# BioJulia/Kmers.jl

Measured on NVIDIA B200. Metric: canonical 31-mers+hash/sec, higher is better.
Workload: dtype u64

## Files before the change

### kmers.jl_b200/csrc/api.cu

```cuda
#include <algorithm>
#include <cstdio>
#include <cstring>
#include <new>
#include <vector>

#include "fourbit.h"
#include "plan.h"

namespace kmc {

int32_t fail_cuda(kmc_ctx *ctx, cudaError_t e, const char *what)
{
    if (ctx) {
        char buf[512];
        snprintf(buf, sizeof buf, "%s: %s (%s)", what, cudaGetErrorName(e), cudaGetErrorString(e));
        ctx->last_error = buf;
    }
    return -static_cast<int32_t>(e);
}

int32_t fail(kmc_ctx *ctx, int32_t code, const char *msg)
{
    if (ctx) ctx->last_error = msg;
    return code;
}

ExtractLaunchFn get_launcher(const Geometry &ge, int mode, bool hash, bool ragged)
{
    switch (ge.n_limbs) {
    case 1: return get_extract_launcher_n1(ge.nx, mode, hash, ragged);
    case 2: return get_extract_launcher_n2(ge.nx, mode, hash, ragged);
    case 3: return get_extract_launcher_n3(ge.nx, mode, hash, ragged);
    case 4: return get_extract_launcher_n4(ge.nx, mode, hash, ragged);
    }
    return nullptr;
}

ExtractLaunchFn get_digest_launcher(const Geometry &ge, int mode, bool hash, bool ragged)
{
    switch (ge.n_limbs) {
    case 1: return get_digest_launcher_n1(ge.nx, mode, hash, ragged);
    case 2: return get_digest_launcher_n2(ge.nx, mode, hash, ragged);
    }
    return nullptr;
}

namespace {

bool aligned32(const void *p) { return (reinterpret_cast<uintptr_t>(p) & 31) == 0; }

__global__ void fill_uniform_offsets_kernel(uint64_t *out, uint64_t n_plus_1, uint64_t step)
{
    uint64_t i = static_cast<uint64_t>(blockIdx.x) * blockDim.x + threadIdx.x;
    if (i < n_plus_1) out[i] = i * step;
}

}

cudaError_t fill_uniform_offsets(uint64_t *out, uint64_t n_plus_1, uint64_t step, cudaStream_t stream)
{
    fill_uniform_offsets_kernel<<<static_cast<unsigned>((n_plus_1 + 255) / 256), 256, 0, stream>>>(out, n_plus_1, step);
    return cudaGetLastError();
}

int32_t check_common(kmc_ctx *ctx, const kmc_seqs *s, int32_t k)
{
    if (!ctx) return KMC_E_BAD_ARG;
    if (!s) return fail(ctx, KMC_E_BAD_ARG, "kmc_seqs is NULL");
    if (k < 1) return fail(ctx, KMC_E_BAD_K, "K must be at least 1");
    if (k > KMC_MAX_K) return fail(ctx, KMC_E_BAD_K, "K exceeds KMC_MAX_K (128)");
    if (s->src_bits != 2 && s->src_bits != 4 && s->src_bits != 8)
        return fail(ctx, KMC_E_BAD_ARG, "src_bits must be 2, 4 (LongSequence words) or 8 (ASCII bytes)");
    if (s->n_seqs > 0 && s->words == nullptr && s->n_words > 0) return fail(ctx, KMC_E_BAD_ARG, "words is NULL");
    return KMC_OK;
}

uint64_t layout_scratch_bytes(const kmc_seqs *s)
{
    if (s->seq_len == nullptr) return 0;
    const uint64_t n = s->n_seqs;
    return 4 * round_up((n + 1) * 8, 256) + round_up(scan_tmp_elems(n) * 8, 256) +
           round_up((tiles_upper_bound(s) + 1) * 8, 256);
}

int32_t plan_layout(kmc_ctx *ctx, const kmc_seqs *s, int k, const Geometry &ge, cudaStream_t stream,
                    const KnownTotals &known, Scratch &scratch, Layout *L)
{
    L->uniform_len = (s->seq_len == nullptr);
    L->uniform_off = (s->seq_word_offset == nullptr);
    const uint64_t G = static_cast<uint64_t>(ge.g);
    if (L->uniform_len) {
        L->wpr = s->uniform_len >= static_cast<uint64_t>(k) ? s->uniform_len - k + 1 : 0;
        L->total = L->wpr * s->n_seqs;
        L->gprm = (L->wpr % G == 0) ? L->wpr / G : (L->wpr + G - 1) / G + 1;
        if (s->n_seqs == 1) L->gprm = (L->wpr + G - 1) / G;
        L->items = L->gprm * s->n_seqs;
        return KMC_OK;
    }
    const uint64_t n = s->n_seqs;
    uint64_t *cnt = static_cast<uint64_t *>(scratch.take((n + 1) * 8));
    uint64_t *win_off = static_cast<uint64_t *>(scratch.take((n + 1) * 8));
    uint64_t *slots = static_cast<uint64_t *>(scratch.take((n + 1) * 8));
    uint64_t *item_off = static_cast<uint64_t *>(scratch.take((n + 1) * 8));
    uint64_t *tmp = static_cast<uint64_t *>(scratch.take(scan_tmp_elems(n) * 8));
    if (!cnt || !win_off || !slots || !item_off || !tmp) return fail(ctx, KMC_E_BAD_ARG, "internal: scratch window too small");
    CU(window_counts(s->seq_len, n, k, cnt, stream));
    CU(inclusive_offsets_u64(cnt, win_off, n, tmp, stream));
    CU(group_slots(win_off, n, ge.g, slots, stream));
    CU(inclusive_offsets_u64(slots, item_off, n, tmp, stream));
    L->win_off = win_off;
    L->item_off = item_off;
    L->wpr = 0;
    L->gprm = 1;
    if (known.valid) {
        L->total = known.windows;
        L->items = known.items;
    } else {
        uint64_t h[2] = {0, 0};
        CU(cudaMemcpyAsync(&h[0], win_off + n, sizeof(uint64_t), cudaMemcpyDeviceToHost, stream));
        CU(cudaMemcpyAsync(&h[1], item_off + n, sizeof(uint64_t), cudaMemcpyDeviceToHost, stream));
        CU(cudaStreamSynchronize(stream));
        L->total = h[0];
        L->items = h[1];
    }
    const uint64_t tiles = (L->items + kTileItems - 1) / kTileItems;
    if (tiles) {
        uint64_t *tile_first = static_cast<uint64_t *>(scratch.take((tiles + 1) * 8));
        if (!tile_first) return fail(ctx, KMC_E_BAD_ARG, "internal: scratch window too small");
        CU(tile_first_reads(item_off, n, kTileItems, tiles, tile_first, stream));
        L->tile_first = tile_first;
    }
    return KMC_OK;
}

ExtractParams base_params(const kmc_seqs *s, int k, const Geometry &ge, const Layout &L, uint64_t unit_bias)
{
    ExtractParams p;
    memset(&p, 0, sizeof p);
    p.w32 = reinterpret_cast<const uint32_t *>(s->words);
    p.nw32 = static_cast<int64_t>(s->n_words) * 2;
    p.unit_bits = 64;
    p.unit_bias = unit_bias;
    p.first = s->first_symbol_offset;
    p.k = k;
    p.s0 = ge.s0;
    p.head_mask = ge.head_mask;
    p.n_seqs = s->n_seqs;
    p.items = L.items;
    p.stride_units = s->uniform_stride_words;
    p.wpr = L.wpr;
    p.gprm = L.gprm;
    p.seq_unit_off = s->seq_word_offset;
    p.win_off = L.win_off;
    p.item_off = L.item_off;
    p.tile_first = L.tile_first;
    return p;
}

int32_t bind_outputs(kmc_ctx *ctx, const kmc_out *out, int mode, uint32_t flags, ExtractParams *p)
{
    const bool hash = (flags & KMC_HASH_FX) != 0;
    const bool aos = (flags & KMC_AOS) != 0;
    const bool want_index = (mode == KMC_UNAMBIG);
    if (!out->a) return fail(ctx, KMC_E_BAD_ARG, "out.a is NULL");
    if (mode == KMC_FWRV && !aos && !out->b) return fail(ctx, KMC_E_BAD_ARG, "out.b is NULL (FWRV, SoA)");
    if (hash && !out->hash) return fail(ctx, KMC_E_BAD_ARG, "out.hash is NULL (KMC_HASH_FX)");
    if (want_index && !aos && !out->index) return fail(ctx, KMC_E_BAD_ARG, "out.index is NULL (UNAMBIG, SoA)");
    p->out_a = out->a;
    p->out_b = out->b;
    p->out_hash = hash ? out->hash : nullptr;
    p->out_index = want_index ? (aos ? reinterpret_cast<int64_t *>(out->a) : out->index) : nullptr;
    p->index_base = out->index_base;
    p->aos = aos ? 1u : 0u;
    p->vec_ok = aligned32(out->a) && (!p->out_b || aligned32(p->out_b)) && (!p->out_hash || aligned32(p->out_hash)) &&
                (!p->out_index || aligned32(p->out_index));
    return KMC_OK;
}

uint64_t extract_scratch_bytes(const kmc_seqs *s, int k, int mode)
{
    if (s->src_bits != 2) return fourbit_scratch_bytes(s, k, mode);
    return layout_scratch_bytes(s) + 256;
}

int32_t extract_device(kmc_ctx *ctx, const kmc_seqs *s, int32_t k, int32_t mode, uint32_t flags, const kmc_out *out,
                       kmc_result *res, cudaStream_t stream, const KnownTotals &known, uint64_t unit_bias, bool sync,
                       Scratch &scratch)
{
    const Geometry ge = geometry(k);
    const bool hash = (flags & KMC_HASH_FX) != 0;
    const int kmode = (mode == KMC_UNAMBIG) ? MODE_FW : mode;

    if (sync) CU(cudaEventRecord(ctx->ev_k0, stream));
    if ((flags & KMC_AOS) && (mode == KMC_FWRV || mode == KMC_UNAMBIG) && ge.n_limbs == 1 && !s->seq_len && !s->seq_word_offset) {
        const Geometry g2 = geometry(k, 2, kAosGroup);
        Layout L2;
        int32_t st2 = plan_layout(ctx, s, k, g2, stream, known, scratch, &L2);
        if (st2) return st2;
        AosLaunchFn afn = get_aos_launcher_n1(g2.nx, mode == KMC_FWRV, hash);
        if (afn && L2.total > 0 && L2.total <= out->capacity) {
            ExtractParams p2 = base_params(s, k, g2, L2, unit_bias);
            st2 = bind_outputs(ctx, out, mode, flags, &p2);
            if (st2) return st2;
            const cudaError_t e = afn(p2, stream);
            if (e == cudaSuccess) {
                res->n_written = L2.total;
                if (out->seq_out_offset) CU(fill_uniform_offsets(out->seq_out_offset, s->n_seqs + 1, L2.wpr, stream));
                if (sync) {
                    CU(cudaEventRecord(ctx->ev_k1, stream));
                    CU(cudaStreamSynchronize(stream));
                    CU(cudaEventElapsedTime(&res->kernel_ms, ctx->ev_k0, ctx->ev_k1));
                }
                return KMC_OK;
            }
            if (e != cudaErrorNotSupported) return fail_cuda(ctx, e, "launch_extract_aos");
            (void)cudaGetLastError();
        }
    }
    Layout L;
    int32_t st = plan_layout(ctx, s, k, ge, stream, known, scratch, &L);
    if (st) return st;
    res->n_written = L.total;
    if (out->seq_out_offset) {
        if (L.uniform_len)
            CU(fill_uniform_offsets(out->seq_out_offset, s->n_seqs + 1, L.wpr, stream));
        else
            CU(cudaMemcpyAsync(out->seq_out_offset, L.win_off, (s->n_seqs + 1) * sizeof(uint64_t), cudaMemcpyDeviceToDevice, stream));
    }
    if (L.total == 0) return KMC_OK;
    if (L.total > out->capacity) return fail(ctx, KMC_E_OUT_TOO_SMALL, "output capacity smaller than the number of k-mers");
    ExtractParams p = base_params(s, k, ge, L, unit_bias);
    st = bind_outputs(ctx, out, mode, flags, &p);
    if (st) return st;

    const bool fused_digest = known.digest && digest_fusable(s, ge.n_limbs, mode, flags);
    if (fused_digest) p.digest = known.digest;
    ExtractLaunchFn fn = fused_digest ? get_digest_launcher(ge, kmode, hash, !L.uniform_len) : get_launcher(ge, kmode, hash, !L.uniform_len);
    if (!fn) return fail(ctx, KMC_E_UNSUPPORTED, "no kernel for this K");
    CU(fn(p, ctx->sm_count, stream));
    if (sync) {
        CU(cudaEventRecord(ctx->ev_k1, stream));
        CU(cudaStreamSynchronize(stream));
        CU(cudaEventElapsedTime(&res->kernel_ms, ctx->ev_k0, ctx->ev_k1));
    }
    return KMC_OK;
}

int32_t ensure_scratch(kmc_ctx *ctx, uint64_t bytes)
{
    if (bytes <= ctx->scratch_bytes) return KMC_OK;
    if (ctx->scratch) {
        CU(cudaStreamSynchronize(ctx->stream));
        for (int i = 0; i < 3; ++i) CU(cudaStreamSynchronize(ctx->pipe_streams[i]));
        CU(cudaFree(ctx->scratch));
        ctx->scratch = nullptr;
        ctx->scratch_bytes = 0;
    }
    uint64_t want = bytes + bytes / 4 + 4096;
    CU(cudaMalloc(&ctx->scratch, want));
    ctx->scratch_bytes = want;
    return KMC_OK;
}

int32_t ensure_host_small(kmc_ctx *ctx)
{
    if (ctx->host_small) return KMC_OK;
    CU(cudaHostAlloc(reinterpret_cast<void **>(&ctx->host_small), 4096, cudaHostAllocDefault));
    memset(ctx->host_small, 0, 4096);
    CU(cudaMalloc(reinterpret_cast<void **>(&ctx->dev_small), 128));
    return KMC_OK;
}

}

using namespace kmc;

extern "C" {

int32_t kmc_version(void) { return KMC_VERSION; }

int32_t kmc_device_count(int32_t *n)
{
    if (!n) return KMC_E_BAD_ARG;
    int c = 0;
    cudaError_t e = cudaGetDeviceCount(&c);
    if (e != cudaSuccess) {
        *n = 0;
        return (e == cudaErrorNoDevice || e == cudaErrorInsufficientDriver) ? KMC_E_NO_DEVICE : -static_cast<int32_t>(e);
    }
    *n = c;
    return KMC_OK;
}

int32_t kmc_ctx_create(int32_t device, kmc_ctx **out)
{
    if (!out) return KMC_E_BAD_ARG;
    *out = nullptr;
    int32_t n = 0;
    int32_t st = kmc_device_count(&n);
    if (st) return st;
    if (n == 0 || device < 0 || device >= n) return KMC_E_NO_DEVICE;
    kmc_ctx *ctx = new (std::nothrow) kmc_ctx();
    if (!ctx) return KMC_E_BAD_ARG;
    ctx->device = device;
    cudaError_t e = cudaSetDevice(device);
    if (e == cudaSuccess) e = cudaDeviceGetAttribute(&ctx->sm_count, cudaDevAttrMultiProcessorCount, device);
    if (e == cudaSuccess) {
        cudaMemPoolProps props;
        memset(&props, 0, sizeof props);
        props.allocType = cudaMemAllocationTypePinned;
        props.handleTypes = cudaMemHandleTypeNone;
        props.location.type = cudaMemLocationTypeDevice;
        props.location.id = device;
        if (cudaMemPoolCreate(&ctx->pool, &props) == cudaSuccess) {
            uint64_t keep = ~0ull;
            cudaMemPoolSetAttribute(ctx->pool, cudaMemPoolAttrReleaseThreshold, &keep);
        } else {
            ctx->pool = nullptr;
        }
        (void)cudaGetLastError();
    }
    if (e == cudaSuccess) e = cudaStreamCreateWithFlags(&ctx->own_stream, cudaStreamNonBlocking);
    for (int i = 0; i < 3 && e == cudaSuccess; ++i) e = cudaStreamCreateWithFlags(&ctx->pipe_streams[i], cudaStreamNonBlocking);
    if (e == cudaSuccess) e = cudaEventCreate(&ctx->ev_begin);
    if (e == cudaSuccess) e = cudaEventCreate(&ctx->ev_end);
    if (e == cudaSuccess) e = cudaEventCreate(&ctx->ev_k0);
    if (e == cudaSuccess) e = cudaEventCreate(&ctx->ev_k1);
    if (e != cudaSuccess) {
        delete ctx;
        return -static_cast<int32_t>(e);
    }
    ctx->stream = ctx->own_stream;
    *out = ctx;
    return KMC_OK;
}

int32_t kmc_ctx_destroy(kmc_ctx *ctx)
{
    if (!ctx) return KMC_OK;
    cudaSetDevice(ctx->device);
    cudaStreamSynchronize(ctx->stream);
    if (ctx->scratch) cudaFree(ctx->scratch);
    if (ctx->host_small) cudaFreeHost(ctx->host_small);
    if (ctx->dev_small) cudaFree(ctx->dev_small);
    for (int i = 0; i < 3; ++i) {
        if (ctx->pipe_buf[i]) cudaFree(ctx->pipe_buf[i]);
        if (ctx->pipe_streams[i]) cudaStreamDestroy(ctx->pipe_streams[i]);
        if (ctx->pipe_events[i]) cudaEventDestroy(ctx->pipe_events[i]);
    }
    if (ctx->ev_begin) cudaEventDestroy(ctx->ev_begin);
    if (ctx->ev_end) cudaEventDestroy(ctx->ev_end);
    if (ctx->ev_k0) cudaEventDestroy(ctx->ev_k0);
    if (ctx->ev_k1) cudaEventDestroy(ctx->ev_k1);
    if (ctx->comm) comm_detach(ctx);
    if (ctx->own_stream) cudaStreamDestroy(ctx->own_stream);
    if (ctx->pool) cudaMemPoolDestroy(ctx->pool);
    delete ctx;
    return KMC_OK;
}

int32_t kmc_ctx_set_stream(kmc_ctx *ctx, void *cuda_stream)
{
    if (!ctx) return KMC_E_BAD_ARG;
    ctx->stream = cuda_stream ? static_cast<cudaStream_t>(cuda_stream) : ctx->own_stream;
    return KMC_OK;
}

int32_t kmc_sync(kmc_ctx *ctx)
{
    if (!ctx) return KMC_E_BAD_ARG;
    CU(cudaSetDevice(ctx->device));
    CU(cudaStreamSynchronize(ctx->stream));
    return KMC_OK;
}

int32_t kmc_trim(kmc_ctx *ctx)
{
    if (!ctx) return KMC_E_BAD_ARG;
    CU(cudaSetDevice(ctx->device));
    CU(cudaStreamSynchronize(ctx->stream));
    for (int i = 0; i < 3; ++i) CU(cudaStreamSynchronize(ctx->pipe_streams[i]));
    if (ctx->pool) CU(cudaMemPoolTrimTo(ctx->pool, 0));
    return KMC_OK;
}

const char *kmc_last_error(kmc_ctx *ctx) { return ctx ? ctx->last_error.c_str() : "kmc_ctx is NULL"; }

const char *kmc_status_string(int32_t status)
{
    switch (status) {
    case KMC_OK: return "ok";
    case KMC_E_BAD_K: return "K must be at least 1 (and at most KMC_MAX_K)";
    case KMC_E_BAD_ARG: return "bad argument";
    case KMC_E_AMBIGUOUS: return "cannot encode an uncertain symbol in a 2-bit alphabet";
    case KMC_E_OUT_TOO_SMALL: return "output buffer too small";
    case KMC_E_NO_DEVICE: return "no CUDA device";
    case KMC_E_UNSUPPORTED: return "unsupported configuration";
    case KMC_E_NCCL: return "NCCL error (or NCCL could not be loaded)";
    }
    if (status < 0) return cudaGetErrorString(static_cast<cudaError_t>(-status));
    return "unknown status";
}

int32_t kmc_device_info(kmc_ctx *ctx, int32_t *sm_count, uint64_t *total_mem, char *name, int32_t name_len)
{
    if (!ctx) return KMC_E_BAD_ARG;
    cudaDeviceProp prop;
    CU(cudaGetDeviceProperties(&prop, ctx->device));
    if (sm_count) *sm_count = prop.multiProcessorCount;
    if (total_mem) *total_mem = prop.totalGlobalMem;
    if (name && name_len > 0) {
        strncpy(name, prop.name, static_cast<size_t>(name_len) - 1);
        name[name_len - 1] = 0;
    }
    return KMC_OK;
}

int32_t kmc_malloc(kmc_ctx *ctx, uint64_t bytes, void **dptr)
{
    if (!ctx || !dptr) return KMC_E_BAD_ARG;
    CU(cudaSetDevice(ctx->device));
    CU(cudaMalloc(dptr, bytes ? bytes : 1));
    return KMC_OK;
}

int32_t kmc_free(kmc_ctx *ctx, void *dptr)
{
    if (!ctx) return KMC_E_BAD_ARG;
    if (!dptr) return KMC_OK;
    CU(cudaSetDevice(ctx->device));
    CU(cudaFree(dptr));
    return KMC_OK;
}

int32_t kmc_memset(kmc_ctx *ctx, void *dptr, int32_t value, uint64_t bytes)
{
    if (!ctx) return KMC_E_BAD_ARG;
    if (bytes == 0) return KMC_OK;
    CU(cudaSetDevice(ctx->device));
    CU(cudaMemsetAsync(dptr, value, bytes, ctx->stream));
    return KMC_OK;
}

int32_t kmc_upload(kmc_ctx *ctx, void *dptr, const void *host, uint64_t bytes)
{
    if (!ctx) return KMC_E_BAD_ARG;
    if (bytes == 0) return KMC_OK;
    CU(cudaSetDevice(ctx->device));
    CU(cudaMemcpyAsync(dptr, host, bytes, cudaMemcpyHostToDevice, ctx->stream));
    return KMC_OK;
}

int32_t kmc_download(kmc_ctx *ctx, void *host, const void *dptr, uint64_t bytes)
{
    if (!ctx) return KMC_E_BAD_ARG;
    CU(cudaSetDevice(ctx->device));
    if (bytes) CU(cudaMemcpyAsync(host, dptr, bytes, cudaMemcpyDeviceToHost, ctx->stream));
    CU(cudaStreamSynchronize(ctx->stream));
    return KMC_OK;
}

int32_t kmc_host_alloc(kmc_ctx *ctx, uint64_t bytes, void **hptr)
{
    if (!ctx || !hptr) return KMC_E_BAD_ARG;
    CU(cudaSetDevice(ctx->device));
    CU(cudaHostAlloc(hptr, bytes ? bytes : 1, cudaHostAllocDefault));
    return KMC_OK;
}

int32_t kmc_host_free(kmc_ctx *ctx, void *hptr)
{
    if (!ctx) return KMC_E_BAD_ARG;
    if (!hptr) return KMC_OK;
    CU(cudaFreeHost(hptr));
    return KMC_OK;
}

int32_t kmc_host_register(kmc_ctx *ctx, void *hptr, uint64_t bytes)
{
    if (!ctx || !hptr) return KMC_E_BAD_ARG;
    CU(cudaSetDevice(ctx->device));
    CU(cudaHostRegister(hptr, bytes, cudaHostRegisterDefault));
    return KMC_OK;
}

int32_t kmc_host_unregister(kmc_ctx *ctx, void *hptr)
{
    if (!ctx || !hptr) return KMC_E_BAD_ARG;
    CU(cudaHostUnregister(hptr));
    return KMC_OK;
}

int32_t kmc_count(kmc_ctx *ctx, const kmc_seqs *seqs, int32_t k, int32_t mode, uint64_t *n_out)
{
    int32_t st = check_common(ctx, seqs, k);
    if (st) return st;
    if (!n_out) return fail(ctx, KMC_E_BAD_ARG, "n_out is NULL");
    if (mode < KMC_FW || mode > KMC_UNAMBIG) return fail(ctx, KMC_E_BAD_ARG, "unknown mode");
    CU(cudaSetDevice(ctx->device));
    if (mode == KMC_UNAMBIG && seqs->src_bits != 2) return count_unambiguous_4bit(ctx, seqs, k, n_out, ctx->stream);
    const Geometry ge = geometry(k);
    st = ensure_scratch(ctx, layout_scratch_bytes(seqs) + 256);
    if (st) return st;
    Scratch scratch{static_cast<char *>(ctx->scratch), ctx->scratch_bytes, 0};
    Layout L;
    st = plan_layout(ctx, seqs, k, ge, ctx->stream, KnownTotals(), scratch, &L);
    if (st) return st;
    *n_out = L.total;
    return KMC_OK;
}

int32_t kmc_extract(kmc_ctx *ctx, const kmc_seqs *seqs, int32_t k, int32_t mode, uint32_t flags, const kmc_out *out,
                    kmc_result *result)
{
    int32_t st = check_common(ctx, seqs, k);
    if (st) return st;
    if (!out || !result) return fail(ctx, KMC_E_BAD_ARG, "kmc_out / kmc_result is NULL");
    if (mode < KMC_FW || mode > KMC_UNAMBIG) return fail(ctx, KMC_E_BAD_ARG, "unknown mode");
    CU(cudaSetDevice(ctx->device));
    result->n_written = 0;
    result->err_seq = result->err_pos = 0;
    result->err_sym = 0;
    result->kernel_ms = 0.f;
    if (flags & KMC_KMER4) {
        st = check_kmer4(ctx, seqs, k, mode);
        if (st) return st;
        st = ensure_scratch(ctx, kmer4_scratch_bytes(seqs));
        if (st) return st;
        Scratch scratch{static_cast<char *>(ctx->scratch), ctx->scratch_bytes, 0};
        return extract_device_kmer4(ctx, seqs, k, mode, flags, out, result, ctx->stream, KnownTotals(), 0,
                                    (flags & KMC_NO_SYNC) == 0, scratch);
    }
    if (seqs->src_bits != 2) return extract_device_4bit(ctx, seqs, k, mode, flags, out, result, ctx->stream);
    st = ensure_scratch(ctx, extract_scratch_bytes(seqs, k, mode));
    if (st) return st;
    Scratch scratch{static_cast<char *>(ctx->scratch), ctx->scratch_bytes, 0};
    return extract_device(ctx, seqs, k, mode, flags, out, result, ctx->stream, KnownTotals(), 0,
                          (flags & KMC_NO_SYNC) == 0, scratch);
}

int32_t kmc_fx_hash(kmc_ctx *ctx, const uint64_t *kmers, uint64_t n, int32_t n_limbs, uint64_t h0, uint64_t *out)
{
    if (!ctx) return KMC_E_BAD_ARG;
    if (n_limbs < 0 || n_limbs > 4) return fail(ctx, KMC_E_BAD_ARG, "n_limbs must be in 0..4");
    if (n && (!out || (n_limbs && !kmers))) return fail(ctx, KMC_E_BAD_ARG, "NULL buffer");
    CU(cudaSetDevice(ctx->device));
    CU(launch_fx_hash(kmers, n, n_limbs, h0, out, ctx->sm_count, ctx->stream));
    return KMC_OK;
}

int32_t kmc_base_hash(kmc_ctx *ctx, const uint64_t *kmers, uint64_t n, int32_t n_limbs, int32_t k, uint64_t h0, uint64_t *out)
{
    if (!ctx) return KMC_E_BAD_ARG;
    if (n_limbs < 0 || n_limbs > 4) return fail(ctx, KMC_E_BAD_ARG, "n_limbs must be in 0..4");
    if (k < 0) return fail(ctx, KMC_E_BAD_K, "K must not be negative");
    if (n && (!out || (n_limbs && !kmers))) return fail(ctx, KMC_E_BAD_ARG, "NULL buffer");
    CU(cudaSetDevice(ctx->device));
    CU(launch_base_hash(kmers, n, n_limbs, h0 ^ static_cast<uint64_t>(k), out, ctx->sm_count, ctx->stream));
    return KMC_OK;
}

namespace {
int32_t bucket_count_impl(kmc_ctx *ctx, const kmc_seqs *seqs, int32_t k, int32_t bucket_bits, uint32_t *table, uint32_t n_parts,
                          void *const *events, kmc_result *result);
}

int32_t kmc_bucket_count(kmc_ctx *ctx, const kmc_seqs *seqs, int32_t k, int32_t bucket_bits, uint32_t *table,
                         kmc_result *result)
{
    return bucket_count_impl(ctx, seqs, k, bucket_bits, table, 0, nullptr, result);
}

int32_t kmc_bucket_count_async(kmc_ctx *ctx, const kmc_seqs *seqs, int32_t k, int32_t bucket_bits, uint32_t *table,
                               uint32_t n_parts, void *const *events, kmc_result *result)
{
    if (!ctx) return KMC_E_BAD_ARG;
    if (!events || n_parts < 1 || n_parts > 32 || (n_parts & (n_parts - 1)))
        return fail(ctx, KMC_E_BAD_ARG, "n_parts must be a power of two <= 32 and events non-NULL");
    for (uint32_t i = 0; i < n_parts; ++i)
        if (!events[i]) return fail(ctx, KMC_E_BAD_ARG, "NULL event");
    return bucket_count_impl(ctx, seqs, k, bucket_bits, table, n_parts, events, result);
}

namespace {
int32_t bucket_count_impl(kmc_ctx *ctx, const kmc_seqs *seqs, int32_t k, int32_t bucket_bits, uint32_t *table, uint32_t n_parts,
                          void *const *events, kmc_result *result)
{
    int32_t st = check_common(ctx, seqs, k);
    if (st) return st;
    if (!table || !result) return fail(ctx, KMC_E_BAD_ARG, "table / result is NULL");
    if (bucket_bits < 1 || bucket_bits > 32) return fail(ctx, KMC_E_BAD_ARG, "bucket_bits must be in 1..32");
    if (seqs->src_bits != 2) return fail(ctx, KMC_E_UNSUPPORTED, "bucket count needs a 2-bit source");
    CU(cudaSetDevice(ctx->device));
    result->n_written = 0;
    result->err_seq = result->err_pos = 0;
    result->err_sym = 0;
    result->kernel_ms = 0.f;
    const Geometry ge = geometry(k);
    cudaStream_t stream = ctx->stream;
    CU(cudaEventRecord(ctx->ev_k0, stream));
    st = ensure_scratch(ctx, layout_scratch_bytes(seqs) + 256);
    if (st) return st;
    Scratch scratch{static_cast<char *>(ctx->scratch), ctx->scratch_bytes, 0};
    Layout L;
    st = plan_layout(ctx, seqs, k, ge, stream, KnownTotals(), scratch, &L);
    if (st) return st;
    result->n_written = L.total;
    auto record_all = [&]() -> int32_t {
        for (uint32_t i = 0; i < n_parts; ++i) CU(cudaEventRecord(static_cast<cudaEvent_t>(events[i]), stream));
        return KMC_OK;
    };
    if (L.total == 0) return record_all();
    ExtractParams p = base_params(seqs, k, ge, L, 0);
    p.bucket_shift = static_cast<uint32_t>(64 - bucket_bits);
    const uint64_t table_bytes = 4ull << bucket_bits;
    const bool want_binned = table_bytes > (96ull << 20) && bucket_bits <= 32;

    auto count_direct = [&](ExtractParams q, cudaStream_t s) -> int32_t {
        int32_t rc = ensure_host_small(ctx);
        if (rc) return rc;
        if (table_bytes <= (96ull << 20)) CU(warm_table(table, 1ull << bucket_bits, ctx->sm_count, warm_sink(ctx), s));
        q.bucket_table = table;
        ExtractLaunchFn fn = get_launcher(ge, MODE_BUCKETS, true, !L.uniform_len);
        if (!fn) return fail(ctx, KMC_E_UNSUPPORTED, "no kernel for this K");
        CU(fn(q, ctx->sm_count, s));
        return KMC_OK;
    };
    auto count_exact = [&](ExtractParams q, uint64_t windows, cudaStream_t s, uint32_t np, void *const *ev) -> int32_t {
        AsyncBuf ids_buf, tmp_buf, matrix_buf, offs_buf, scan_buf;
        const uint64_t n_ids = (q.items + 1) * static_cast<uint64_t>(ge.g);
        const uint64_t cells = (static_cast<uint64_t>(1) << binned_count_bin_bits(bucket_bits)) * binned_count_blocks(n_ids);
        cudaError_t e = ids_buf.alloc(ctx, round_up(n_ids * 4, 256), s);
        if (e == cudaSuccess) e = tmp_buf.alloc(ctx, round_up(n_ids * 4, 256), s);
        if (e == cudaSuccess) e = matrix_buf.alloc(ctx, (cells + 1) * 8, s);
        if (e == cudaSuccess) e = offs_buf.alloc(ctx, (cells + 2) * 8, s);
        if (e == cudaSuccess) e = scan_buf.alloc(ctx, (scan_tmp_elems(cells) + 1) * 8, s);
        if (e != cudaSuccess) {
            (void)cudaGetLastError();
            int32_t rc = count_direct(q, s);
            if (rc) return rc;
            for (uint32_t i = 0; i < np; ++i) CU(cudaEventRecord(static_cast<cudaEvent_t>(ev[i]), s));
            return KMC_OK;
        }
        q.out_a = ids_buf.as<uint64_t>();
        q.vec_ok = 1;
        ExtractLaunchFn fn = get_launcher(ge, MODE_BUCKET_IDS, true, !L.uniform_len);
        if (!fn) return fail(ctx, KMC_E_UNSUPPORTED, "no kernel for this K");
        CU(fn(q, ctx->sm_count, s));
        CU(binned_count(ids_buf.as<uint32_t>(), windows, bucket_bits, table, tmp_buf.as<uint32_t>(), matrix_buf.as<uint64_t>(),
                        offs_buf.as<uint64_t>(), scan_buf.as<uint64_t>(), ctx->sm_count, s, np, ev));
        return KMC_OK;
    };

    bool done = false;
    ExtractParams pa = p;
    if (want_binned) set_iteration_strides(pa, ge.g);
    if (want_binned && ge.n_limbs == 1 && L.uniform_len && binned_count_bin_bits(bucket_bits) == 6 && fused_bin_enabled() && pa.aligned &&
        pa.al_tail == 0 && pa.items < 0xffffffffull - kTileItems) {
        AsyncBuf bins_buf, state_buf;
        const uint64_t cap = fused_bin_capacity(L.total);
        cudaError_t e = bins_buf.alloc(ctx, fused_bin_buffer_ids(L.total) * 4, stream);
        if (e == cudaSuccess) e = state_buf.alloc(ctx, fused_bin_state_bytes(), stream);
        if (e != cudaSuccess) {
            (void)cudaGetLastError();
        } else {
            st = ensure_host_small(ctx);
            if (st) return st;
            CU(fused_bin_ids(pa, ge.nx, bucket_bits, bins_buf.as<uint32_t>(), cap, state_buf.as<unsigned long long>(), stream));
            CU(fused_bin_apply(bins_buf.as<uint32_t>(), cap, state_buf.as<unsigned long long>(), bucket_bits, table, warm_sink(ctx),
                               ctx->sm_count, stream, n_parts, events));
            done = true;
        }
    }
    if (!done && want_binned) {
        st = count_exact(p, L.total, stream, n_parts, events);
        if (st) return st;
        done = true;
    }
    if (!done) {
        st = count_direct(p, stream);
        if (st) return st;
        st = record_all();
        if (st) return st;
    }
    if (n_parts) return KMC_OK;
    CU(cudaEventRecord(ctx->ev_k1, stream));
    CU(cudaStreamSynchronize(stream));
    CU(cudaEventElapsedTime(&result->kernel_ms, ctx->ev_k0, ctx->ev_k1));
    return KMC_OK;
}
}

int32_t kmc_digest(kmc_ctx *ctx, const uint64_t *dptr, uint64_t n, uint64_t *out)
{
    if (!ctx) return KMC_E_BAD_ARG;
    if (!out || (n && !dptr)) return fail(ctx, KMC_E_BAD_ARG, "NULL buffer");
    CU(cudaSetDevice(ctx->device));
    int32_t st = ensure_scratch(ctx, 256);
    if (st) return st;
    uint64_t *acc = static_cast<uint64_t *>(ctx->scratch);
    CU(launch_digest(dptr, n, acc, ctx->sm_count, ctx->stream));
    CU(cudaMemcpyAsync(out, acc, 16, cudaMemcpyDeviceToHost, ctx->stream));
    CU(cudaStreamSynchronize(ctx->stream));
    return KMC_OK;
}

int32_t kmc_timer_begin(kmc_ctx *ctx)
{
    if (!ctx) return KMC_E_BAD_ARG;
    CU(cudaSetDevice(ctx->device));
    CU(cudaEventRecord(ctx->ev_begin, ctx->stream));
    return KMC_OK;
}

int32_t kmc_timer_end(kmc_ctx *ctx, float *ms)
{
    if (!ctx || !ms) return KMC_E_BAD_ARG;
    CU(cudaSetDevice(ctx->device));
    CU(cudaEventRecord(ctx->ev_end, ctx->stream));
    CU(cudaEventSynchronize(ctx->ev_end));
    CU(cudaEventElapsedTime(ms, ctx->ev_begin, ctx->ev_end));
    return KMC_OK;
}

int32_t kmc_store_probe(kmc_ctx *ctx, void *dptr, uint64_t bytes)
{
    if (!ctx || !dptr) return KMC_E_BAD_ARG;
    CU(cudaSetDevice(ctx->device));
    CU(launch_store_probe(dptr, bytes, ctx->sm_count, ctx->stream));
    return KMC_OK;
}

}
```

### kmers.jl_b200/csrc/buckets.cu

```cuda
#include <cstdlib>
#include <type_traits>

#include "binning.cuh"
#include "plan.h"

namespace kmc {

namespace {

__global__ void __launch_bounds__(256) warm_slice_kernel(const uint32_t *__restrict__ slice, uint64_t n_counters,
                                                         uint32_t *__restrict__ sink)
{
    const uint4 *p = reinterpret_cast<const uint4 *>(slice);
    const uint64_t n4 = n_counters / 4;
    uint32_t acc = 0;
    for (uint64_t i = static_cast<uint64_t>(blockIdx.x) * blockDim.x + threadIdx.x; i < n4;
         i += static_cast<uint64_t>(gridDim.x) * blockDim.x) {
        uint4 v;
        asm volatile("ld.global.L1::no_allocate.L2::cache_hint.v4.u32 {%0,%1,%2,%3}, [%4], %5;"
                     : "=r"(v.x), "=r"(v.y), "=r"(v.z), "=r"(v.w)
                     : "l"(p + i), "l"(0x14F0000000000000ull));
        acc |= v.x & v.y & v.z & v.w;
    }
    if (acc == 0xffffffffu) *sink = acc;
}

__global__ void __launch_bounds__(256) bin_apply_kernel(const uint32_t *__restrict__ binned, const uint64_t *__restrict__ offs,
                                                        uint64_t n_blocks, int bin, int bin_end, uint32_t *__restrict__ table)
{
    const uint64_t begin = __ldg(offs + static_cast<uint64_t>(bin) * n_blocks);
    const uint64_t end = __ldg(offs + static_cast<uint64_t>(bin_end) * n_blocks);
    const uint64_t a4 = (begin + 3) & ~3ull;
    const uint64_t tid = static_cast<uint64_t>(blockIdx.x) * blockDim.x + threadIdx.x;
    const uint64_t threads = static_cast<uint64_t>(gridDim.x) * blockDim.x;
    if (tid < a4 - begin && begin + tid < end) atomicAdd(table + binned[begin + tid], 1u);
    for (uint64_t i = a4 + tid * 4; i < end; i += threads * 4) {
        if (i + 4 <= end) {
            const uint4 v = __ldg(reinterpret_cast<const uint4 *>(binned + i));
            atomicAdd(table + v.x, 1u);
            atomicAdd(table + v.y, 1u);
            atomicAdd(table + v.z, 1u);
            atomicAdd(table + v.w, 1u);
        } else {
            for (uint64_t j = i; j < end; ++j) atomicAdd(table + binned[j], 1u);
        }
    }
}


constexpr int kStateBinEnd = binning::kTpBins;
constexpr int kStateSpill = 2 * binning::kTpBins;
constexpr int kStateWords = 2 * binning::kTpBins + 2;

struct FusedBins {
    uint32_t *binned;
    uint64_t cap;
    unsigned long long *state;
    int bin_shift;
};

template <int NX>
__global__ void __launch_bounds__(binning::kBlock, 3) bucket_bin_kernel(const ExtractParams p, const FusedBins f)
{
    using S = binning::Shape<uint32_t>;
    constexpr int G = 8, PT = S::kPerThread;
    static_assert(PT == 2 * G && S::kChunk == kTileItems * G, "a thread bins the ids of two work items per iteration");
    extern __shared__ __align__(16) unsigned char smem_raw[];
    binning::Scatter64Smem<uint32_t> &sm = *reinterpret_cast<binning::Scatter64Smem<uint32_t> *>(smem_raw);
    const uint32_t n_items = static_cast<uint32_t>(p.items);
    const uint32_t tile_base = blockIdx.x * static_cast<uint32_t>(kTileItems);
    if (p.pf_tiles) burst_prefetch<false, G, 2>(p, n_items);
    const AlignedItems<G, 2> items(p);
    const uint32_t tile_end = n_items - tile_base > static_cast<uint32_t>(kTileItems) ? tile_base + kTileItems : n_items;
    const bool inside = items.template loads_inside<NX>(p, tile_end - 1u);
    const binning::IdBin bin_of{f.bin_shift};
    constexpr int kItemsPerIter = 2 * binning::kBlock;
    auto reserve = [&](int b, uint32_t count) -> uint64_t {
        if (count == 0) return 0;
        const uint64_t at = atomicAdd(f.state + b, static_cast<unsigned long long>(count));
        if (at + count > f.cap) {
            atomicMin(f.state + kStateBinEnd + b, static_cast<unsigned long long>(at));
            return binning::kTpBins * f.cap + atomicAdd(f.state + kStateSpill, static_cast<unsigned long long>(count));
        }
        return static_cast<uint64_t>(b) * f.cap + at;
    };
    auto ids_of = [&](uint32_t item, uint32_t *key) {
        uint32_t x[NX];
        load_block_at<NX>(p, items.bit_of(item), inside, x);
        uint64_t fw[G][1], rv[G][1];
        block_kmers<1, NX, G, true, true, 2>(x, p.s0, p.head_mask, fw, rv);
#pragma unroll
        for (int j = 0; j < G; ++j) {
            const uint64_t c[1] = {fw[j][0] < rv[j][0] ? fw[j][0] : rv[j][0]};
            key[j] = static_cast<uint32_t>(fx_hash<1>(c, 0) >> p.bucket_shift);
        }
    };
#pragma unroll 1
    for (uint32_t it_base = tile_base; it_base < tile_end; it_base += kItemsPerIter) {
        uint32_t key[PT];
        if (tile_end - it_base >= static_cast<uint32_t>(kItemsPerIter)) {
            ids_of(it_base + threadIdx.x, key);
            ids_of(it_base + binning::kBlock + threadIdx.x, key + G);
            binning::scatter64_iter<uint32_t, true>(sm, key, 0xffffu, bin_of, reserve, f.binned);
        } else {
            uint32_t ok_mask = 0;
#pragma unroll
            for (int j = 0; j < PT; ++j) key[j] = 0;
            if (it_base + threadIdx.x < tile_end) {
                ids_of(it_base + threadIdx.x, key);
                ok_mask = 0xffu;
            }
            if (it_base + binning::kBlock + threadIdx.x < tile_end) {
                ids_of(it_base + binning::kBlock + threadIdx.x, key + G);
                ok_mask |= 0xff00u;
            }
            binning::scatter64_iter<uint32_t, false>(sm, key, ok_mask, bin_of, reserve, f.binned);
        }
    }
}

__device__ __forceinline__ uint4 ld_ids(const uint32_t *p)
{
    uint4 v;
    asm volatile("ld.global.nc.L1::no_allocate.L2::cache_hint.v4.u32 {%0,%1,%2,%3}, [%4], %5;"
                 : "=r"(v.x), "=r"(v.y), "=r"(v.z), "=r"(v.w)
                 : "l"(p), "l"(0x12F0000000000000ull));
    return v;
}
__device__ __forceinline__ void inc_counter(uint32_t *p)
{
    asm volatile("red.global.add.L2::cache_hint.u32 [%0], 1, %1;" ::"l"(p), "l"(0x14F0000000000000ull) : "memory");
}

__global__ void __launch_bounds__(256) bin_apply_fused_kernel(const uint32_t *__restrict__ binned, uint64_t cap,
                                                              const unsigned long long *__restrict__ state, int bin, int bin_end,
                                                              uint32_t *__restrict__ table)
{
    const uint64_t tid = static_cast<uint64_t>(blockIdx.x) * blockDim.x + threadIdx.x;
    const uint64_t step = static_cast<uint64_t>(gridDim.x) * blockDim.x * 4;
    for (int b = bin; b < bin_end; ++b) {
        const uint32_t *ids = binned + static_cast<uint64_t>(b) * cap;
        const uint64_t reserved = state[b], full_at = state[kStateBinEnd + b];
        const uint64_t n = reserved < full_at ? reserved : full_at, n4 = n & ~3ull;
        uint64_t i = tid * 4;
        uint4 v = make_uint4(0, 0, 0, 0);
        if (i < n4) v = ld_ids(ids + i);
        while (i < n4) {
            const uint64_t nxt = i + step;
            uint4 w = make_uint4(0, 0, 0, 0);
            if (nxt < n4) w = ld_ids(ids + nxt);
            inc_counter(table + v.x);
            inc_counter(table + v.y);
            inc_counter(table + v.z);
            inc_counter(table + v.w);
            v = w;
            i = nxt;
        }
        if (tid < n - n4) inc_counter(table + ids[n4 + tid]);
    }
}

__global__ void __launch_bounds__(256) spill_apply_kernel(const uint32_t *__restrict__ spill, const unsigned long long *__restrict__ state,
                                                          uint32_t *__restrict__ table)
{
    const uint64_t n = state[kStateSpill];
    for (uint64_t i = static_cast<uint64_t>(blockIdx.x) * blockDim.x + threadIdx.x; i < n; i += static_cast<uint64_t>(gridDim.x) * blockDim.x)
        atomicAdd(table + spill[i], 1u);
}

}

cudaError_t binned_count(const uint32_t *ids, uint64_t n, int bucket_bits, uint32_t *table, uint32_t *binned, uint64_t *matrix,
                         uint64_t *offs, uint64_t *scan_tmp, int sm_count, cudaStream_t stream, uint32_t n_parts, void *const *events)
{
    if (!events) n_parts = 0;
    if (n == 0) {
        for (uint32_t i = 0; i < n_parts; ++i) {
            cudaError_t e = cudaEventRecord(static_cast<cudaEvent_t>(events[i]), stream);
            if (e != cudaSuccess) return e;
        }
        return cudaSuccess;
    }
    const int p = binned_count_bin_bits(bucket_bits);
    if (bucket_bits < p) return cudaErrorInvalidValue;
    const int n_bins = 1 << p, shift = bucket_bits - p;
    const uint64_t n_blocks = binned_count_blocks(n);
    cudaError_t e = binning::partition<uint32_t>(ids, n, p, binning::IdBin{shift}, binned, matrix, offs, scan_tmp, stream);
    if (e != cudaSuccess) return e;
    const uint64_t slice = 1ull << shift;
    const int group = apply_group(2);
    uint32_t parts_done = 0;
    for (int b = 0; b < n_bins; b += group) {
        const int b_end = b + group < n_bins ? b + group : n_bins;
        warm_slice_kernel<<<static_cast<unsigned>(sm_count * 8), 256, 0, stream>>>(table + static_cast<uint64_t>(b) * slice,
                                                                                  slice * (b_end - b), reinterpret_cast<uint32_t *>(scan_tmp));
        bin_apply_kernel<<<static_cast<unsigned>(sm_count * 16), 256, 0, stream>>>(binned, offs, n_blocks, b, b_end, table);
        while (parts_done < n_parts && static_cast<uint64_t>(parts_done + 1) * n_bins <= static_cast<uint64_t>(b_end) * n_parts) {
            e = cudaEventRecord(static_cast<cudaEvent_t>(events[parts_done++]), stream);
            if (e != cudaSuccess) return e;
        }
    }
    return cudaGetLastError();
}

uint64_t fused_bin_capacity(uint64_t n_ids)
{
    const uint64_t cap = n_ids / binning::kTpBins + n_ids / (8 * binning::kTpBins) + 8192;
    return (cap + 3) & ~3ull;
}
uint64_t fused_bin_buffer_ids(uint64_t n_ids) { return binning::kTpBins * fused_bin_capacity(n_ids) + n_ids + 4096; }
uint64_t fused_bin_state_bytes() { return kStateWords * sizeof(unsigned long long); }

cudaError_t fused_bin_ids(ExtractParams p, int nx, int bucket_bits, uint32_t *binned, uint64_t cap, unsigned long long *state,
                          cudaStream_t stream)
{
    const int pbits = binned_count_bin_bits(bucket_bits);
    if (pbits != 6 || bucket_bits < pbits) return cudaErrorInvalidValue;
    const uint64_t tiles = (p.items + kTileItems - 1) / kTileItems;
    if (tiles == 0 || tiles > 0x7fffffffull || p.items >= 0xffffffffull - kTileItems) return cudaErrorInvalidConfiguration;
    set_iteration_strides(p, 8);
    if (!p.aligned || p.al_tail) return cudaErrorInvalidValue;
    p.al_magic = aligned_magic(p.gprm);
    p.pf_tiles = 0;
    if (prefetch_enabled()) {
        const uint64_t per_tile = static_cast<uint64_t>(p.nw32) * 4 / tiles + 1, t = kPfChunkBytes / per_tile;
        p.pf_tiles = static_cast<uint32_t>(t < 2 * kPfLead ? 2 * kPfLead : (t > (1u << 20) ? (1u << 20) : t));
    }
    cudaError_t e = cudaMemsetAsync(state, 0, kStateWords * sizeof(unsigned long long), stream);
    if (e == cudaSuccess) e = cudaMemsetAsync(state + kStateBinEnd, 0xff, binning::kTpBins * sizeof(unsigned long long), stream);
    if (e != cudaSuccess) return e;
    const FusedBins f{binned, cap, state, bucket_bits - pbits};
    constexpr int smem = static_cast<int>(sizeof(binning::Scatter64Smem<uint32_t>));
    auto launch = [&](auto tag) -> cudaError_t {
        constexpr int NX = decltype(tag)::value;
        cudaError_t e2 = cudaFuncSetAttribute(bucket_bin_kernel<NX>, cudaFuncAttributeMaxDynamicSharedMemorySize, smem);
        if (e2 != cudaSuccess) return e2;
        bucket_bin_kernel<NX><<<static_cast<unsigned>(tiles), binning::kBlock, smem, stream>>>(p, f);
        return cudaGetLastError();
    };
    switch (nx) {
    case 1: return launch(std::integral_constant<int, 1>());
    case 2: return launch(std::integral_constant<int, 2>());
    case 3: return launch(std::integral_constant<int, 3>());
    }
    return cudaErrorInvalidValue;
}

cudaError_t fused_bin_apply(const uint32_t *binned, uint64_t cap, const unsigned long long *state, int bucket_bits, uint32_t *table,
                            uint32_t *sink, int sm_count, cudaStream_t stream, uint32_t n_parts, void *const *events)
{
    if (!events) n_parts = 0;
    const int pbits = binned_count_bin_bits(bucket_bits);
    const int n_bins = 1 << pbits, shift = bucket_bits - pbits;
    const uint64_t slice = 1ull << shift;
    const int group = apply_group(2);
    spill_apply_kernel<<<static_cast<unsigned>(sm_count * 8), 256, 0, stream>>>(binned + static_cast<uint64_t>(n_bins) * cap, state, table);
    uint32_t parts_done = 0;
    for (int b = 0; b < n_bins; b += group) {
        const int b_end = b + group < n_bins ? b + group : n_bins;
        warm_slice_kernel<<<static_cast<unsigned>(sm_count * 8), 256, 0, stream>>>(table + static_cast<uint64_t>(b) * slice,
                                                                                  slice * (b_end - b), sink);
        bin_apply_fused_kernel<<<static_cast<unsigned>(sm_count * 16), 256, 0, stream>>>(binned, cap, state, b, b_end, table);
        while (parts_done < n_parts && static_cast<uint64_t>(parts_done + 1) * n_bins <= static_cast<uint64_t>(b_end) * n_parts) {
            cudaError_t e = cudaEventRecord(static_cast<cudaEvent_t>(events[parts_done++]), stream);
            if (e != cudaSuccess) return e;
        }
    }
    return cudaGetLastError();
}

bool fused_bin_enabled()
{
    static const bool on = [] {
        const char *e = getenv("KMC_FUSED_BIN");
        return !(e && e[0] == '0');
    }();
    return on;
}

int apply_group(int dflt)
{
    static const int env = [] {
        const char *e = getenv("KMC_APPLY_GROUP");
        const int v = e ? atoi(e) : 0;
        return v < 0 ? 0 : (v > 64 ? 64 : v);
    }();
    return env ? env : dflt;
}

cudaError_t warm_table(const uint32_t *table, uint64_t n_counters, int sm_count, uint32_t *sink, cudaStream_t stream)
{
    warm_slice_kernel<<<static_cast<unsigned>(sm_count * 8), 256, 0, stream>>>(table, n_counters, sink);
    return cudaGetLastError();
}

int binned_count_bin_bits(int bucket_bits)
{
    int p = bucket_bits - 22;
    if (p < binning::kMinBits) p = binning::kMinBits;
    if (p > binning::kMaxBits) p = binning::kMaxBits;
    return p;
}

uint64_t binned_count_blocks(uint64_t n) { return binning::blocks_for<uint32_t>(n); }

}
```

### kmers.jl_b200/csrc/kmc_internal.h

```cpp
#pragma once
#include <cuda_runtime.h>
#include <cstdint>
#include <string>

#include "../../include/kmerscuda.h"

struct kmc_comm;

struct kmc_ctx {
    int device = 0;
    int sm_count = 0;
    cudaStream_t own_stream = nullptr;
    cudaStream_t stream = nullptr;
    cudaStream_t pipe_streams[3] = {nullptr, nullptr, nullptr};
    cudaEvent_t pipe_events[3] = {nullptr, nullptr, nullptr};
    cudaEvent_t ev_begin = nullptr, ev_end = nullptr;
    cudaEvent_t ev_k0 = nullptr, ev_k1 = nullptr;
    void *scratch = nullptr;
    uint64_t scratch_bytes = 0;
    void *pipe_buf[3] = {nullptr, nullptr, nullptr};
    uint64_t pipe_bytes[3] = {0, 0, 0};
    uint64_t *host_small = nullptr;
    uint64_t *dev_small = nullptr;
    cudaMemPool_t pool = nullptr;
    kmc_comm *comm = nullptr;
    std::string last_error;
};

namespace kmc {

struct AsyncBuf {
    void *p = nullptr;
    cudaStream_t s = nullptr;
    cudaError_t alloc(kmc_ctx *ctx, uint64_t bytes, cudaStream_t stream)
    {
        s = stream;
        return ctx->pool ? cudaMallocFromPoolAsync(&p, bytes ? bytes : 1, ctx->pool, stream)
                         : cudaMallocAsync(&p, bytes ? bytes : 1, stream);
    }
    template <typename T> T *as() const { return static_cast<T *>(p); }
    AsyncBuf() = default;
    AsyncBuf(const AsyncBuf &) = delete;
    AsyncBuf &operator=(const AsyncBuf &) = delete;
    ~AsyncBuf()
    {
        if (p) cudaFreeAsync(p, s);
    }
};

inline uint32_t *warm_sink(kmc_ctx *ctx) { return reinterpret_cast<uint32_t *>(ctx->dev_small) + 24; }

void comm_detach(kmc_ctx *ctx);

int32_t ensure_scratch(kmc_ctx *ctx, uint64_t bytes);
int32_t ensure_host_small(kmc_ctx *ctx);

uint64_t scan_tmp_elems(uint64_t n);
cudaError_t inclusive_offsets_u64(const uint64_t *in, uint64_t *out, uint64_t n, uint64_t *tmp, cudaStream_t stream);
cudaError_t window_counts(const uint64_t *seq_len, uint64_t n, int k, uint64_t *cnt, cudaStream_t stream);
cudaError_t group_slots(const uint64_t *win_off, uint64_t n, int g, uint64_t *slots, cudaStream_t stream);

cudaError_t tile_first_reads(const uint64_t *item_off, uint64_t n_seqs, uint64_t tile_items, uint64_t n_tiles,
                             uint64_t *tile_first, cudaStream_t stream);

int binned_count_bin_bits(int bucket_bits);
int apply_group(int dflt);
uint64_t binned_count_blocks(uint64_t n);
cudaError_t warm_table(const uint32_t *table, uint64_t n_counters, int sm_count, uint32_t *sink, cudaStream_t stream);
cudaError_t binned_count(const uint32_t *ids, uint64_t n, int bucket_bits, uint32_t *table, uint32_t *binned, uint64_t *matrix,
                         uint64_t *offs, uint64_t *scan_tmp, int sm_count, cudaStream_t stream, uint32_t n_parts = 0,
                         void *const *events = nullptr);

struct ExtractParams;
bool fused_bin_enabled();
uint64_t fused_bin_capacity(uint64_t n_ids);
uint64_t fused_bin_buffer_ids(uint64_t n_ids);
uint64_t fused_bin_state_bytes();
cudaError_t fused_bin_ids(ExtractParams p, int nx, int bucket_bits, uint32_t *binned, uint64_t cap, unsigned long long *state,
                          cudaStream_t stream);
cudaError_t fused_bin_apply(const uint32_t *binned, uint64_t cap, const unsigned long long *state, int bucket_bits, uint32_t *table,
                            uint32_t *sink, int sm_count, cudaStream_t stream, uint32_t n_parts, void *const *events);

cudaError_t launch_fx_hash(const uint64_t *kmers, uint64_t n, int n_limbs, uint64_t h0, uint64_t *out, int sm_count,
                           cudaStream_t stream);
cudaError_t launch_digest(const uint64_t *p, uint64_t n, uint64_t *acc, int sm_count, cudaStream_t stream, bool zero = true);
cudaError_t launch_base_hash(const uint64_t *kmers, uint64_t n, int n_limbs, uint64_t h, uint64_t *out, int sm_count,
                             cudaStream_t stream);
cudaError_t launch_store_probe(void *dptr, uint64_t bytes, int sm_count, cudaStream_t stream);

}
```

Baseline: 454.6 billion.

## Add two-level sub-binning with shared-memory counting for fused bin apply

Adds a second partition pass that splits each coarse bin into 32K-counter sub-bins and stores 16-bit offsets. A new count kernel then accumulates each sub-bin in a 128KB shared-memory histogram and adds it to the global table slice with a single vectorized read-modify-write. This replaces scattered global atomics on the table with shared-memory atomics and coalesced writes. The cost is an extra pass over the ids, an extra buffer allocation, and a possible overflow spill path. The new path is enabled by default through an environment flag.

```diff
diff --git a/kmers.jl_b200/csrc/api.cu b/kmers.jl_b200/csrc/api.cu
--- a/kmers.jl_b200/csrc/api.cu
+++ b/kmers.jl_b200/csrc/api.cu
@@ -664,11 +664,21 @@
         if (e != cudaSuccess) {
             (void)cudaGetLastError();
         } else {
+            AsyncBuf sub_buf;
+            bool smem = smem_count_enabled() && (reinterpret_cast<uintptr_t>(table) & 15) == 0;
+            if (smem && sub_buf.alloc(ctx, sub_bin_buffer_bytes(L.total, bucket_bits), stream) != cudaSuccess) {
+                (void)cudaGetLastError();
+                smem = false;
+            }
             st = ensure_host_small(ctx);
             if (st) return st;
             CU(fused_bin_ids(pa, ge.nx, bucket_bits, bins_buf.as<uint32_t>(), cap, state_buf.as<unsigned long long>(), stream));
-            CU(fused_bin_apply(bins_buf.as<uint32_t>(), cap, state_buf.as<unsigned long long>(), bucket_bits, table, warm_sink(ctx),
-                               ctx->sm_count, stream, n_parts, events));
+            if (smem)
+                CU(fused_sub_count(bins_buf.as<uint32_t>(), cap, state_buf.as<unsigned long long>(), bucket_bits, table, sub_buf.p, L.total,
+                                   ctx->sm_count, stream, n_parts, events));
+            else
+                CU(fused_bin_apply(bins_buf.as<uint32_t>(), cap, state_buf.as<unsigned long long>(), bucket_bits, table, warm_sink(ctx),
+                                   ctx->sm_count, stream, n_parts, events));
             done = true;
         }
     }
diff --git a/kmers.jl_b200/csrc/buckets.cu b/kmers.jl_b200/csrc/buckets.cu
--- a/kmers.jl_b200/csrc/buckets.cu
+++ b/kmers.jl_b200/csrc/buckets.cu
@@ -168,6 +168,183 @@
         atomicAdd(table + spill[i], 1u);
 }
 
+constexpr int kSubBits = 15, kSubCounters = 1 << kSubBits;
+constexpr int kSplitBlock = 256, kSplitPT = 16, kSplitTile = kSplitBlock * kSplitPT;
+constexpr int kMaxSubPerBin = 128;
+constexpr int kCountBlock = 1024;
+
+struct SubBins {
+    uint16_t *offs;
+    uint64_t cap;
+    unsigned long long *state;
+    int n_sub;
+};
+
+struct SplitSmem {
+    uint32_t ids[kSplitTile];
+    uint32_t cnt[kMaxSubPerBin];
+    uint32_t start[kMaxSubPerBin];
+    uint64_t dst[kMaxSubPerBin];
+    uint32_t spilled[kMaxSubPerBin];
+};
+
+__global__ void __launch_bounds__(kSplitBlock, 4) sub_split_kernel(uint32_t *__restrict__ binned, uint64_t cap,
+                                                                   unsigned long long *__restrict__ state, uint64_t tiles_per_bin,
+                                                                   const SubBins s)
+{
+    __shared__ SplitSmem sm;
+    const uint32_t per_bin = static_cast<uint32_t>(s.n_sub) / binning::kTpBins, sub_mask = per_bin - 1u;
+    uint32_t *spill = binned + binning::kTpBins * cap;
+    for (uint64_t t = blockIdx.x; t < binning::kTpBins * tiles_per_bin; t += gridDim.x) {
+        const int b = static_cast<int>(t / tiles_per_bin);
+        const uint64_t base = (t % tiles_per_bin) * kSplitTile;
+        const uint64_t reserved = state[b], full_at = state[kStateBinEnd + b];
+        const uint64_t n = reserved < full_at ? reserved : full_at;
+        if (base >= n) continue;
+        const uint32_t m = n - base < static_cast<uint64_t>(kSplitTile) ? static_cast<uint32_t>(n - base) : kSplitTile;
+        const uint32_t *src = binned + static_cast<uint64_t>(b) * cap + base;
+        if (threadIdx.x < per_bin) sm.cnt[threadIdx.x] = 0;
+        __syncthreads();
+        uint32_t id[kSplitPT], rank[kSplitPT / 2];
+        uint32_t ok = 0;
+#pragma unroll
+        for (int r = 0; r < kSplitPT / 4; ++r) {
+            const uint32_t e = r * (4 * kSplitBlock) + threadIdx.x * 4;
+            if (e + 4 <= m) {
+                const uint4 v = ld_ids(src + e);
+                id[4 * r] = v.x;
+                id[4 * r + 1] = v.y;
+                id[4 * r + 2] = v.z;
+                id[4 * r + 3] = v.w;
+                ok |= 0xfu << (4 * r);
+            } else {
+#pragma unroll
+                for (int q = 0; q < 4; ++q) {
+                    const bool in = e + q < m;
+                    id[4 * r + q] = in ? src[e + q] : 0u;
+                    ok |= (in ? 1u : 0u) << (4 * r + q);
+                }
+            }
+        }
+#pragma unroll
+        for (int j = 0; j < kSplitPT; ++j) {
+            const uint32_t r = ((ok >> j) & 1u) ? atomicAdd(&sm.cnt[(id[j] >> kSubBits) & sub_mask], 1u) : 0u;
+            rank[j / 2] = (j % 2 == 0) ? r : (rank[j / 2] | (r << 16));
+        }
+        __syncthreads();
+        uint32_t c = 0;
+        uint64_t at = 0;
+        if (threadIdx.x < per_bin) {
+            c = sm.cnt[threadIdx.x];
+            if (c) at = atomicAdd(s.state + static_cast<uint64_t>(b) * per_bin + threadIdx.x, static_cast<unsigned long long>(c));
+        }
+        if (threadIdx.x < 32) {
+            const int lane = threadIdx.x;
+            uint32_t cq[4], sum = 0;
+#pragma unroll
+            for (int q = 0; q < 4; ++q) {
+                cq[q] = 4 * lane + q < static_cast<int>(per_bin) ? sm.cnt[4 * lane + q] : 0u;
+                sum += cq[q];
+            }
+            uint32_t incl = sum;
+#pragma unroll
+            for (int d = 1; d < 32; d <<= 1) {
+                const uint32_t a = __shfl_up_sync(0xffffffffu, incl, d);
+                if (lane >= d) incl += a;
+            }
+            uint32_t run = incl - sum;
+#pragma unroll
+            for (int q = 0; q < 4; ++q) {
+                if (4 * lane + q < static_cast<int>(per_bin)) sm.start[4 * lane + q] = run;
+                run += cq[q];
+            }
+        }
+        __syncthreads();
+        if (threadIdx.x < per_bin) {
+            const uint64_t g = static_cast<uint64_t>(b) * per_bin + threadIdx.x;
+            uint64_t dst = 0;
+            uint32_t spilled = 0;
+            if (c) {
+                if (at + c > s.cap) {
+                    atomicMin(s.state + s.n_sub + g, static_cast<unsigned long long>(at));
+                    dst = atomicAdd(state + kStateSpill, static_cast<unsigned long long>(c));
+                    spilled = 1;
+                } else {
+                    dst = g * s.cap + at;
+                }
+            }
+            sm.dst[threadIdx.x] = dst - sm.start[threadIdx.x];
+            sm.spilled[threadIdx.x] = spilled;
+        }
+#pragma unroll
+        for (int j = 0; j < kSplitPT; ++j)
+            if ((ok >> j) & 1u) sm.ids[sm.start[(id[j] >> kSubBits) & sub_mask] + ((rank[j / 2] >> (16 * (j % 2))) & 0xffffu)] = id[j];
+        __syncthreads();
+#pragma unroll
+        for (int k = 0; k < kSplitPT; ++k) {
+            const uint32_t i = threadIdx.x + k * kSplitBlock;
+            if (i < m) {
+                const uint32_t v = sm.ids[i], sub = (v >> kSubBits) & sub_mask;
+                const uint64_t d = sm.dst[sub] + i;
+                if (sm.spilled[sub])
+                    spill[d] = v;
+                else
+                    s.offs[d] = static_cast<uint16_t>(v & (kSubCounters - 1));
+            }
+        }
+        __syncthreads();
+    }
+}
+
+__global__ void __launch_bounds__(kCountBlock, 1) sub_count_kernel(const uint16_t *__restrict__ offs, uint64_t cap,
+                                                                   const unsigned long long *__restrict__ sub_state, int n_sub,
+                                                                   uint64_t g0, uint32_t *__restrict__ table)
+{
+    extern __shared__ __align__(16) uint4 smem_cnt[];
+    uint32_t *cnt = reinterpret_cast<uint32_t *>(smem_cnt);
+    const uint64_t g = g0 + blockIdx.x;
+    uint4 *slice = reinterpret_cast<uint4 *>(table + (g << kSubBits));
+    static_assert(kCountBlock * 128 == kSubCounters * 4, "one 128-byte line of the slice per thread");
+    asm volatile("prefetch.global.L2::evict_last [%0];" ::"l"(slice + threadIdx.x * 8));
+#pragma unroll
+    for (int i = 0; i < kSubCounters / 4 / kCountBlock; ++i) smem_cnt[threadIdx.x + i * kCountBlock] = make_uint4(0, 0, 0, 0);
+    __syncthreads();
+    const uint64_t reserved = sub_state[g], full_at = sub_state[n_sub + g];
+    const uint64_t n = reserved < full_at ? reserved : full_at, n8 = n & ~7ull;
+    const uint16_t *ids = offs + g * cap;
+    auto count8 = [&](const uint4 v) {
+        const uint32_t w[4] = {v.x, v.y, v.z, v.w};
+#pragma unroll
+        for (int q = 0; q < 4; ++q) {
+            atomicAdd(cnt + (w[q] & 0xffffu), 1u);
+            atomicAdd(cnt + (w[q] >> 16), 1u);
+        }
+    };
+    constexpr uint64_t kStep = kCountBlock * 8;
+    uint64_t i = threadIdx.x * 8ull;
+    for (; i + 3 * kStep < n8; i += 4 * kStep) {
+        uint4 v[4];
+#pragma unroll
+        for (int u = 0; u < 4; ++u) v[u] = ld_ids(reinterpret_cast<const uint32_t *>(ids + i + u * kStep));
+#pragma unroll
+        for (int u = 0; u < 4; ++u) count8(v[u]);
+    }
+    for (; i < n8; i += kStep) count8(ld_ids(reinterpret_cast<const uint32_t *>(ids + i)));
+    if (threadIdx.x < n - n8) atomicAdd(cnt + ids[n8 + threadIdx.x], 1u);
+    __syncthreads();
+#pragma unroll
+    for (int k = 0; k < kSubCounters / 4 / kCountBlock; ++k) {
+        const int j = threadIdx.x + k * kCountBlock;
+        uint4 t = slice[j];
+        const uint4 c = smem_cnt[j];
+        t.x += c.x;
+        t.y += c.y;
+        t.z += c.z;
+        t.w += c.w;
+        slice[j] = t;
+    }
+}
+
 }
 
 cudaError_t binned_count(const uint32_t *ids, uint64_t n, int bucket_bits, uint32_t *table, uint32_t *binned, uint64_t *matrix,
@@ -269,6 +446,53 @@
     return cudaGetLastError();
 }
 
+uint64_t sub_bin_capacity(uint64_t n_ids, int bucket_bits)
+{
+    const uint64_t n_sub = 1ull << (bucket_bits - kSubBits);
+    const uint64_t cap = n_ids / n_sub + n_ids / (8 * n_sub) + 1024;
+    return (cap + 7) & ~7ull;
+}
+uint64_t sub_bin_buffer_bytes(uint64_t n_ids, int bucket_bits)
+{
+    const uint64_t n_sub = 1ull << (bucket_bits - kSubBits);
+    return 2 * n_sub * sizeof(unsigned long long) + n_sub * sub_bin_capacity(n_ids, bucket_bits) * sizeof(uint16_t);
+}
+
+cudaError_t fused_sub_count(uint32_t *binned, uint64_t cap, unsigned long long *state, int bucket_bits, uint32_t *table, void *sub_buf,
+                            uint64_t n_ids, int sm_count, cudaStream_t stream, uint32_t n_parts, void *const *events)
+{
+    if (!events) n_parts = 0;
+    if (binned_count_bin_bits(bucket_bits) != 6 || bucket_bits - 6 - kSubBits > 7 || bucket_bits - 6 < kSubBits)
+        return cudaErrorInvalidValue;
+    const int n_sub = 1 << (bucket_bits - kSubBits), per_bin = n_sub / binning::kTpBins;
+    SubBins s{nullptr, sub_bin_capacity(n_ids, bucket_bits), static_cast<unsigned long long *>(sub_buf), n_sub};
+    s.offs = reinterpret_cast<uint16_t *>(s.state + 2 * n_sub);
+    cudaError_t e = cudaMemsetAsync(s.state, 0, n_sub * sizeof(unsigned long long), stream);
+    if (e == cudaSuccess) e = cudaMemsetAsync(s.state + n_sub, 0xff, n_sub * sizeof(unsigned long long), stream);
+    if (e == cudaSuccess) e = cudaFuncSetAttribute(sub_count_kernel, cudaFuncAttributeMaxDynamicSharedMemorySize, kSubCounters * 4);
+    if (e != cudaSuccess) return e;
+    const uint64_t tiles_per_bin = (cap + kSplitTile - 1) / kSplitTile;
+    const uint64_t tiles = binning::kTpBins * tiles_per_bin, grid = static_cast<uint64_t>(sm_count) * 4;
+    sub_split_kernel<<<static_cast<unsigned>(tiles < grid ? tiles : grid), kSplitBlock, 0, stream>>>(binned, cap, state, tiles_per_bin, s);
+    spill_apply_kernel<<<static_cast<unsigned>(sm_count * 8), 256, 0, stream>>>(binned + binning::kTpBins * cap, state, table);
+    const int group = binning::kTpBins / static_cast<int>(n_parts ? n_parts : 1);
+    for (int b = 0; b < binning::kTpBins; b += group) {
+        sub_count_kernel<<<static_cast<unsigned>(group * per_bin), kCountBlock, kSubCounters * 4, stream>>>(
+            s.offs, s.cap, s.state, n_sub, static_cast<uint64_t>(b) * per_bin, table);
+        if (n_parts) {
+            e = cudaEventRecord(static_cast<cudaEvent_t>(events[b / group]), stream);
+            if (e != cudaSuccess) return e;
+        }
+    }
+    return cudaGetLastError();
+}
+
+bool smem_count_enabled()
+{
+    const char *e = getenv("KMC_SMEM_COUNT");
+    return !(e && e[0] == '0');
+}
+
 bool fused_bin_enabled()
 {
     static const bool on = [] {
diff --git a/kmers.jl_b200/csrc/kmc_internal.h b/kmers.jl_b200/csrc/kmc_internal.h
--- a/kmers.jl_b200/csrc/kmc_internal.h
+++ b/kmers.jl_b200/csrc/kmc_internal.h
@@ -80,6 +80,10 @@
                           cudaStream_t stream);
 cudaError_t fused_bin_apply(const uint32_t *binned, uint64_t cap, const unsigned long long *state, int bucket_bits, uint32_t *table,
                             uint32_t *sink, int sm_count, cudaStream_t stream, uint32_t n_parts, void *const *events);
+bool smem_count_enabled();
+uint64_t sub_bin_buffer_bytes(uint64_t n_ids, int bucket_bits);
+cudaError_t fused_sub_count(uint32_t *binned, uint64_t cap, unsigned long long *state, int bucket_bits, uint32_t *table, void *sub_buf,
+                            uint64_t n_ids, int sm_count, cudaStream_t stream, uint32_t n_parts, void *const *events);
 
 cudaError_t launch_fx_hash(const uint64_t *kmers, uint64_t n, int n_limbs, uint64_t h0, uint64_t *out, int sm_count,
                            cudaStream_t stream);
```

Result: no change. 454.6 billion, median of 6 (-0.0%).
